# DogRog/no-time-to-train

Hardware: NVIDIA B200
Metric: matching_stage_images_per_s (higher is better)
Workload: dtype f32

## Files before the change

### no-time-to-train_b200/csrc/api.cu

```cuda
#include <cstdio>
#include <cstdlib>
#include <cstring>
#include <mutex>

#include "common.cuh"

namespace nttt {

int launch_lowres_pack(const float*, int, int, int, float, float, uint32_t*, int32_t*, int32_t*, int32_t*, int32_t*,
                       const float*, float, const float* const*, cudaStream_t, float* stab_score = nullptr);
int launch_multimask_select(const float*, int, int, int, const ChunkTable&, int, size_t, const float**, float*,
                            cudaStream_t);
int launch_project_masks(const AxisTable&, const AxisTable&, const uint32_t*, const int32_t*, int, int, int, int, int,
                         void*, int, bool, cudaStream_t, const int32_t* perm = nullptr, uint32_t* active = nullptr);
int launch_pool_order(const int32_t*, int, int, int32_t*, cudaStream_t);
int launch_normalize_split(const float*, int, const int32_t*, int, int, int, float*, void*, bool, cudaStream_t,
                           const int32_t* perm = nullptr);
int launch_gemm_tc(const void*, int, const void*, int, float*, int, int, int, int, int, size_t, int*, cudaStream_t,
                   bool low_latency = false, const uint32_t* a_active = nullptr, const uint8_t* b_nonfinite = nullptr);
int gemm_tc_pick_splits(int, int, int, int);
int launch_split_rows(const float*, int, int, int, int, int, void*, cudaStream_t);
int launch_split_transpose(const float*, int, int, int, int, int, void*, cudaStream_t, uint8_t* nonfinite = nullptr);
int launch_normalize_rows(const float*, int, const int32_t*, int, int, float*, bool, cudaStream_t);
int launch_proto_prepare(const float*, int, int, int, float*, cudaStream_t);
int launch_top1(const float*, int, size_t, float*, int, int, int, float*, int32_t*, cudaStream_t);
int launch_neg_top1(const float*, int, size_t, const float*, int, size_t, int, int, int, float, float*, float*, int32_t*,
                    cudaStream_t);
size_t nms_workspace_bytes(int n);
int launch_box_nms(const int32_t*, const float*, const int32_t*, const float*, int, float, int, int32_t*, int32_t*,
                   int32_t*, int32_t*, void*, size_t, float, int, cudaStream_t);
int launch_upsample_pack(const AxisTable&, const AxisTable&, const float*, const uint32_t*, const int32_t*,
                         const int32_t*, int, int, const int32_t*, const int32_t*, int, int, int, uint32_t*, int32_t*,
                         int32_t*, int32_t*, int32_t*, const float* const*, cudaStream_t, int, int, uint32_t* bits_t = nullptr,
                         bool* wrote_t = nullptr, bool t_only = false, bool low_latency = false, int32_t* zero2 = nullptr);
int32_t* ios_pair_counters(void* ws, int max_sel);
size_t upsample_scratch_bytes(int max_sel, int oh, int ow);
int launch_unpack_sparse(const uint32_t*, const int32_t*, const int32_t*, const int32_t*, int, int, int, uint8_t*,
                         int32_t*, cudaStream_t, bool tr = false);
int launch_unpack(const uint32_t*, const int32_t*, const int32_t*, const int32_t*, int, int, int, uint8_t*,
                  cudaStream_t, bool tr = false);
size_t ios_workspace_bytes(int max_sel);
int launch_mask_ios(const uint32_t*, const int32_t*, const int32_t*, const int32_t*, const int32_t*, const int32_t*,
                    int, int, int, const int32_t*, const float*, int, float*, int32_t*, void*, bool, cudaStream_t,
                    const uint32_t* bits_t = nullptr, bool counters_zeroed = false);
int launch_decay_rank(const float*, const int32_t*, const float*, const int32_t*, const int32_t*, int, int,
                      const int32_t*, const int32_t*, int64_t*, float*, int64_t*, int32_t*, int32_t*, int32_t*, float*,
                      cudaStream_t);
int launch_rle_encode(const uint32_t*, const int32_t*, const int32_t*, const int32_t*, int, int, int, int, int, uint32_t*,
                      int32_t*, uint8_t*, int32_t*, cudaStream_t, bool tr = false);
int launch_rle_compact(const uint8_t*, const int32_t*, int, int, uint8_t*, long long, cudaStream_t);
int launch_fill_pool(const float*, const float*, int, int, int, int, int, int, float*, float*, float*, int, cudaStream_t);
int launch_fill_scatter(const float*, const float*, const float*, const int32_t*, int, int, int, float*, float*, float*,
                        cudaStream_t);
int launch_fill_finalize(const float*, const float*, int, int, int, float*, float*, cudaStream_t);

extern int g_pack_persistent;
static thread_local char g_cuda_err[512] = "";
std::atomic<unsigned long long> g_launches{0};
thread_local bool t_low_latency = false;
thread_local bool t_chain_break = false;

cudaError_t set_dyn_smem_impl(const void* fn, int bytes) {
  struct Entry { const void* fn; int dev; int bytes; };
  static std::mutex mu;
  static Entry table[256];
  static int n = 0;
  int dev = 0;
  cudaError_t e = cudaGetDevice(&dev);
  if (e != cudaSuccess) return e;
  std::lock_guard<std::mutex> lock(mu);
  Entry* hit = nullptr;
  for (int i = 0; i < n; ++i)
    if (table[i].fn == fn && table[i].dev == dev) { hit = &table[i]; break; }
  if (hit && hit->bytes >= bytes) return cudaSuccess;
  e = cudaFuncSetAttribute(fn, cudaFuncAttributeMaxDynamicSharedMemorySize, bytes);
  if (e != cudaSuccess) return e;
  if (hit) hit->bytes = bytes;
  else if (n < 256) table[n++] = Entry{fn, dev, bytes};
  return cudaSuccess;
}

int cuda_fail(cudaError_t e, const char* what) {
  snprintf(g_cuda_err, sizeof(g_cuda_err), "%s: %s (%s)", what, cudaGetErrorString(e), cudaGetErrorName(e));
  return (e == cudaErrorNoDevice || e == cudaErrorInsufficientDriver) ? NTTT_ENODEVICE : NTTT_ECUDA;
}

struct Carver {
  char* base;
  size_t off = 0;
  explicit Carver(void* p) : base(static_cast<char*>(p)) {}
  template <typename T>
  T* take(size_t count) {
    off = align_up(off, 256);
    T* p = base ? reinterpret_cast<T*>(base + off) : nullptr;
    off += sizeof(T) * count;
    return p;
  }
};

inline int pad64(int k) { return (k + 63) / 64 * 64; }

constexpr int kPoolSplitsMax = 2;
constexpr int kPoolSplits = 1;
static int pool_contract(const float* proj, const float* feat, int n, int e, int c, float* sums, void* a_split,
                         void* b_split, int* n_partials, cudaStream_t s, bool low_latency = false, bool b_ready = false,
                         const uint32_t* a_active = nullptr, uint8_t* b_nonfinite = nullptr) {
  const int ep = pad64(e);
  int err = proj ? launch_split_rows(proj, e, n, e, ep, 0, a_split, s) : NTTT_OK;
  if (err) return err;
  err = b_ready ? NTTT_OK : launch_split_transpose(feat, c, c, e, ep, 1, b_split, s, a_active ? b_nonfinite : nullptr);
  if (err) return err;
  return launch_gemm_tc(a_split, 3 * ep, b_split, 3 * ep, sums, c, n, c, 3 * ep, low_latency ? kPoolSplitsMax : kPoolSplits,
                        (size_t)n * c, n_partials, s, low_latency, a_active, a_active ? b_nonfinite : nullptr);
}

static int normalize_rows(const float* sums, int n_partials, const int32_t* area, int n, int c, float* obj_feats,
                          void* a_split, bool* split_done, bool nan_empty, cudaStream_t s, const int32_t* perm = nullptr) {
  *split_done = a_split &&
                launch_normalize_split(sums, n_partials, area, n, c, pad64(c), obj_feats, a_split, nan_empty, s, perm) == 1;
  if (*split_done) return NTTT_OK;
  if (perm) return NTTT_EINVAL;
  return launch_normalize_rows(sums, n_partials, area, n, c, obj_feats, nan_empty, s);
}

static bool projection_supported(int in_size, int out_size) {
  return in_size > 0 && 2 * ((out_size + in_size - 1) / in_size) + 2 <= kMaxScatter;
}

constexpr int kMaxSimSplits = 8;
static size_t sim_partial_floats(int n, int cols, int c) {
  int sp = gemm_tc_pick_splits(n, cols, 3 * pad64(c), 148);
  if (sp > kMaxSimSplits) sp = kMaxSimSplits;
  return (size_t)sp * n * cols;
}

static int sim_top1(const float* obj_feats, const float* proto, const float* proto_neg, int l_neg, float sigma, int n,
                    int c, int n_cls, float* sim, float* partials, float* partials_neg, float* top_score,
                    int32_t* top_label, void* a_split, void* b_split, bool a_ready, int sm_count, cudaStream_t s,
                    void* p_split = nullptr, bool p_ready = false) {
  const int cp = pad64(c);
  int err = a_ready ? NTTT_OK : launch_split_rows(obj_feats, c, n, c, cp, 0, a_split, s);
  if (err) return err;
  void* pb = p_split ? p_split : b_split;
  err = p_ready ? NTTT_OK : launch_split_rows(proto, c, n_cls, c, cp, 1, pb, s);
  if (err) return err;
  int want = gemm_tc_pick_splits(n, n_cls, 3 * cp, sm_count < 148 ? sm_count : 148);
  if (want > kMaxSimSplits) want = kMaxSimSplits;
  if (!t_low_latency) want = 1;
  const size_t stride = (size_t)n * n_cls;
  int splits = 1;
  err = launch_gemm_tc(a_split, 3 * cp, pb, 3 * cp, partials, n_cls, n, n_cls, 3 * cp, want, stride, &splits, s);
  if (err) return err;
  if (!proto_neg) return launch_top1(partials, splits, stride, sim, n_cls, n, n_cls, top_score, top_label, s);
  const int cols = n_cls * l_neg;
  err = launch_split_rows(proto_neg, c, cols, c, cp, 1, b_split, s);
  if (err) return err;
  int want_n = gemm_tc_pick_splits(n, cols, 3 * cp, sm_count < 148 ? sm_count : 148);
  if (want_n > kMaxSimSplits) want_n = kMaxSimSplits;
  if (!t_low_latency) want_n = 1;
  const size_t stride_n = (size_t)n * cols;
  int splits_n = 1;
  err = launch_gemm_tc(a_split, 3 * cp, b_split, 3 * cp, partials_neg, cols, n, cols, 3 * cp, want_n, stride_n, &splits_n,
                       s);
  if (err) return err;
  return launch_neg_top1(partials, splits, stride, partials_neg, splits_n, stride_n, n, n_cls, l_neg, sigma, sim,
                         top_score, top_label, s);
}

// ... 488 lines not shown
  L.sim_part = cv.take<float>(sim_partial_floats(n, n_cls, c));
  L.sim_part_neg = cv.take<float>(l_neg > 0 ? sim_partial_floats(n, n_cls * l_neg, c) : 1);
  {
    const size_t kmax = (size_t)3 * (pad64(eh * ew) > pad64(c) ? pad64(eh * ew) : pad64(c));
    size_t rows_b = (size_t)(c > n_cls ? c : n_cls);
    if ((size_t)n_cls * (l_neg > 0 ? l_neg : 0) > rows_b) rows_b = (size_t)n_cls * l_neg;
    L.a_split = cv.take<char>(2 * (size_t)n * kmax);
    L.b_split = cv.take<char>(2 * rows_b * kmax);
    L.p_split = cv.take<char>(2 * (size_t)n_cls * 3 * pad64(c));
    L.pool_perm = cv.take<int32_t>(n > 0 ? n : 1);
    L.pool_active = cv.take<uint32_t>(n > 0 ? n : 1);
    L.b_nonfinite = cv.take<uint8_t>((size_t)(pad64(eh * ew) / 64) * ((c + 31) / 32));
  }
  L.top_score = cv.take<float>(n);
  L.top_label = cv.take<int32_t>(n);
  L.nms_ws_bytes = nms_workspace_bytes(n > 0 ? n : 1);
  L.nms_ws = cv.take<char>(L.nms_ws_bytes);
  L.keep = cv.take<int32_t>(max_sel > 0 ? max_sel : 1);
  L.sel = cv.take<int32_t>(max_sel > 0 ? max_sel : 1);
  L.bits_full = cv.take<uint32_t>((size_t)max_sel * oh * ((ow + 31) / 32));
  L.bits_t = cv.take<uint32_t>((size_t)max_sel * oh * ((ow + 31) / 32));
  L.rect = cv.take<int32_t>((size_t)max_sel * 4);
  L.area_full = cv.take<int32_t>(max_sel > 0 ? max_sel : 1);
  L.box_full = cv.take<int32_t>((size_t)max_sel * 4);
  L.scratch = cv.take<int32_t>(upsample_scratch_bytes(max_sel > 0 ? max_sel : 1, oh, ow) / sizeof(int32_t) + 1);
  L.ios = cv.take<float>(max_sel > 0 ? max_sel : 1);
  L.ios_ws = cv.take<char>(ios_workspace_bytes(max_sel > 0 ? max_sel : 1));
  L.out_slot = cv.take<int32_t>(num_out > 0 ? num_out : 1);
  L.mask_ptr = cv.take<const float*>(n > 0 ? n : 1);
  L.plane_score = cv.take<float>(n > 0 ? n : 1);
  L.total = align_up(cv.off, 256);
  return L;
}

size_t nttt_match_workspace_bytes(int n, int lr_h, int lr_w, int eh, int ew, int c, int n_cls, int ori_h, int ori_w,
                                  int max_sel) {
  if (n < 0 || lr_h <= 0 || lr_w <= 0 || eh <= 0 || ew <= 0 || c <= 0 || n_cls <= 0 || ori_h <= 0 || ori_w <= 0 ||
      max_sel < 0)
    return 0;
  return carve(nullptr, n, lr_h, lr_w, eh, ew, c, n_cls, ori_h, ori_w, max_sel, max_sel, 0).total;
}

size_t nttt_match_workspace_bytes_neg(int n, int lr_h, int lr_w, int eh, int ew, int c, int n_cls, int ori_h, int ori_w,
                                      int max_sel, int l_neg) {
  if (n < 0 || lr_h <= 0 || lr_w <= 0 || eh <= 0 || ew <= 0 || c <= 0 || n_cls <= 0 || ori_h <= 0 || ori_w <= 0 ||
      max_sel < 0 || l_neg < 0)
    return 0;
  return carve(nullptr, n, lr_h, lr_w, eh, ew, c, n_cls, ori_h, ori_w, max_sel, max_sel, l_neg).total;
}

int nttt_match_image(nttt_ctx* ctx, const nttt_match_args* a, void* stream) {
  if (!ctx || !a) return NTTT_EINVAL;
  if (a->n < 0 || a->lr_h <= 0 || a->lr_w <= 0 || a->eh <= 0 || a->ew <= 0 || a->c <= 0 || a->n_cls <= 0 ||
      a->ori_h <= 0 || a->ori_w <= 0 || a->num_out_instance < 0 || a->max_sel < 0)
    return NTTT_EINVAL;
  if (!a->counts || !a->workspace) return NTTT_EINVAL;
  cudaStream_t s = (cudaStream_t)stream;
  const int n = a->n, max_sel = a->max_sel, num_out = a->num_out_instance;
  if (n == 0 || max_sel == 0) {
    NTTT_CUDA(cudaMemsetAsync(a->counts, 0, 4 * sizeof(int32_t), s));
    return NTTT_OK;
  }
  const bool multi = a->n_multi > 1;
  const bool chunked = multi && a->logits_chunks_host;
  const bool want_rle = a->rle_chars != nullptr;
  if ((!a->logits && !chunked) || (!multi && !a->pred_ious) || !a->tar_feat || !a->proto ||
      (!a->out_masks && !want_rle) || !a->out_boxes || !a->out_scores || !a->out_labels || !a->out_index)
    return NTTT_EINVAL;
  if (want_rle && (!a->rle_counts || !a->rle_n_counts || !a->rle_n_chars || a->rle_cap_counts <= 0 || a->rle_cap_chars <= 0))
    return NTTT_EINVAL;
  if (multi && (!a->multi_ious || a->multi_first < 0 || a->multi_first >= a->n_multi)) return NTTT_EINVAL;
  const int l_neg = a->proto_neg ? a->l_neg : 0;
  if (a->proto_neg && (a->l_neg <= 0 || !(a->sigma > 0.0f))) return NTTT_EINVAL;
  MatchLayout L = carve(a->workspace, n, a->lr_h, a->lr_w, a->eh, a->ew, a->c, a->n_cls, a->ori_h, a->ori_w, max_sel,
                        num_out, l_neg);
  if (a->workspace_bytes < L.total) return NTTT_EWORKSPACE;
  if (!projection_supported(a->ew, a->lr_w) || !projection_supported(a->eh, a->lr_h)) return NTTT_EUNSUPPORTED;
  float* obj_feats = a->obj_feats ? a->obj_feats : L.obj_feats;
  float* sim = a->sim ? a->sim : L.sim;
  int32_t* sel = a->sel ? a->sel : L.sel;
  float* ios = a->ios ? a->ios : L.ios;
  struct LaunchMode {
    bool prev;
    explicit LaunchMode(bool v) : prev(nttt::t_low_latency) { nttt::t_low_latency = v; }
    ~LaunchMode() { nttt::t_low_latency = prev; }
  } launch_mode(a->low_latency != 0);
  ++ctx->epoch;
  AxisTable px, py, ux, uy;
  int err = ctx->axis(a->ew, a->lr_w, s, &px);
  if (err) return err;
  if ((err = ctx->axis(a->eh, a->lr_h, s, &py))) return err;
  if ((err = ctx->axis(a->lr_w, a->ori_w, s, &ux))) return err;
  if ((err = ctx->axis(a->lr_h, a->ori_h, s, &uy))) return err;
  const int e = a->eh * a->ew;

  ctx->n_ev = 0;
#define NTTT_MARK()                                                              \
  do {                                                                           \
    if (ctx->profile) { NTTT_CUDA(cudaEventRecord(ctx->ev[ctx->n_ev], s)); ++ctx->n_ev; } \
  } while (0)
#ifdef NTTT_ABLATE
  int stage_no = 0;
#define NTTT_STOP_CHECK() if (ctx->stop_after > 0 && ++stage_no >= ctx->stop_after) return NTTT_OK
#else
#define NTTT_STOP_CHECK() (void)0
#endif
#define NTTT_STEP_QUIET(call) \
  do {                        \
    err = (call);             \
    if (err) return err;      \
  } while (0)
#define NTTT_STEP(call)                                        \
  do {                                                         \
    err = (call);                                              \
    if (err) return err;                                       \
    NTTT_MARK();                                               \
    NTTT_STOP_CHECK();                                         \
  } while (0)
  const float* const* mask_ptr = nullptr;
  const float* pred_ious = a->pred_ious;
  if (multi) {
    ChunkTable ct;
    const float* one = a->logits;
    err = chunked ? make_chunk_table(a->logits_chunks_host, a->n_chunks, a->chunk_prompts, n, &ct)
                  : make_chunk_table(&one, 1, n, n, &ct);
    if (err) return err;
    if ((err = launch_multimask_select(a->multi_ious, n, a->n_multi, a->multi_first, ct, chunked ? a->chunk_prompts : n,
                                       (size_t)a->lr_h * a->lr_w, L.mask_ptr, L.plane_score, s)))
      return err;
    mask_ptr = L.mask_ptr;
    pred_ious = L.plane_score;
  }
  NTTT_MARK();
  const bool forked = a->low_latency != 0 && ctx->side_ready();
  struct SideJoin {
    cudaStream_t s;
    cudaEvent_t ev = nullptr;
    ~SideJoin() { if (ev) cudaStreamWaitEvent(s, ev, 0); }
  } side_join{s};
  if (forked) {
    NTTT_CUDA(cudaEventRecord(ctx->ev_fork, s));
    NTTT_CUDA(cudaStreamWaitEvent(ctx->side, ctx->ev_fork, 0));
    err = launch_split_transpose(a->tar_feat, a->c, a->c, e, pad64(e), 1, L.b_split, ctx->side);
    if (err) return err;
    err = launch_split_rows(a->proto, a->c, a->n_cls, a->c, pad64(a->c), 1, L.p_split, ctx->side);
    if (err) return err;
    NTTT_CUDA(cudaEventRecord(ctx->ev_join, ctx->side));
    side_join.ev = ctx->ev_join;
  }
  NTTT_STEP(launch_lowres_pack(a->logits, n, a->lr_h, a->lr_w, 0.0f, 1.0f, L.bits_lr, L.area_lr, L.box_lr, nullptr,
                               L.flags, a->filter_iou ? pred_ious : nullptr, a->iou_thr, mask_ptr, s));
  const bool ordered = !a->low_latency && ctx->pool_order && n > 128 && n <= 8192 && pad64(e) / 64 <= 32 &&
                       (a->c == 384 || a->c == 768 || a->c == 1024 || a->c == 1536);
  if (ordered) NTTT_STEP_QUIET(launch_pool_order(L.box_lr, n, a->lr_h, L.pool_perm, s));
  NTTT_STEP(launch_project_masks(px, py, L.bits_lr, L.box_lr, n, a->lr_h, a->lr_w, a->eh, a->ew, L.a_split, pad64(e),
                                 true, s, ordered ? L.pool_perm : nullptr, ordered ? L.pool_active : nullptr));
  int n_partials = 1;
  if (forked) {
    NTTT_CUDA(cudaStreamWaitEvent(s, ctx->ev_join, 0));
    side_join.ev = nullptr;
    nttt::t_chain_break = true;
  }
  NTTT_STEP(pool_contract(nullptr, a->tar_feat, n, e, a->c, L.sums, L.a_split, L.b_split, &n_partials, s,
                          a->low_latency != 0, forked, ordered ? L.pool_active : nullptr, L.b_nonfinite));
  bool a_ready = false;
  NTTT_STEP(normalize_rows(L.sums, n_partials, L.area_lr, n, a->c, obj_feats, L.a_split, &a_ready,
                           a->proto_neg != nullptr, s, ordered ? L.pool_perm : nullptr));
  NTTT_STEP(sim_top1(obj_feats, a->proto, a->proto_neg, l_neg, a->sigma, n, a->c, a->n_cls, a->sim, L.sim_part,
                     L.sim_part_neg, L.top_score, L.top_label, L.a_split, L.b_split, a_ready, ctx->sm_count, s, L.p_split,
                     forked));
  NTTT_STEP(launch_box_nms(L.box_lr, pred_ious, L.top_label, L.top_score, n, a->nms_thr, max_sel, L.keep,
                           a->counts + 0, sel, a->counts + 1, L.nms_ws, L.nms_ws_bytes, a->iou_thr, a->filter_iou, s));
  bool wrote_t = false;
  NTTT_STEP(launch_upsample_pack(ux, uy, a->logits, L.bits_lr, L.box_lr, L.flags, a->lr_h, a->lr_w, sel,
                                 a->counts + 1, max_sel, a->ori_h, a->ori_w, L.bits_full, L.rect, L.area_full,
                                 L.box_full, L.scratch, mask_ptr, s, ctx->upsample_stage_floats, ctx->sm_count, L.bits_t,
                                 &wrote_t, true, a->low_latency != 0, ios_pair_counters(L.ios_ws, max_sel)));
  const uint32_t* packed = wrote_t ? L.bits_t : L.bits_full;
  NTTT_STEP(launch_mask_ios(L.bits_full, L.rect, L.area_full, L.box_full, sel, a->counts + 1, max_sel, a->ori_h,
                            a->ori_w, L.top_label, obj_feats, a->c, ios, a->ios_inter, L.ios_ws, false, s,
                            wrote_t ? L.bits_t : nullptr, wrote_t && a->low_latency != 0));
  NTTT_STEP(launch_decay_rank(L.top_score, L.top_label, ios, sel, a->counts + 1, max_sel, num_out, L.box_full,
                              L.area_full,
                              a->out_boxes, a->out_scores, a->out_labels, a->out_index, L.out_slot, a->counts + 2,
                              nullptr, s));
  if (!a->out_masks)
    NTTT_MARK();
  else if (a->out_prev_rect)
    NTTT_STEP(launch_unpack_sparse(packed, L.rect, L.out_slot, a->counts + 2, num_out, a->ori_h, a->ori_w,
                                   a->out_masks, a->out_prev_rect, s, wrote_t));
  else
    NTTT_STEP(launch_unpack(packed, L.rect, L.out_slot, a->counts + 2, num_out, a->ori_h, a->ori_w, a->out_masks,
                            s, wrote_t));
  if (want_rle)
    NTTT_STEP(launch_rle_encode(packed, L.rect, L.out_slot, a->counts + 2, num_out, a->ori_h, a->ori_w,
                                a->rle_cap_counts, a->rle_cap_chars, a->rle_counts, a->rle_n_counts, a->rle_chars,
                                a->rle_n_chars, s, wrote_t));
  else
    NTTT_MARK();
#undef NTTT_STEP
#undef NTTT_STOP_CHECK
#undef NTTT_MARK
  return NTTT_OK;
}

}
```

### no-time-to-train_b200/csrc/lowres.cu

```cuda
#include <cuda_bf16.h>
#include <stdlib.h>

#include <algorithm>

#include "common.cuh"

namespace nttt {

constexpr int kPackThreads = 256;
constexpr int kPackBlock = kPackThreads + 32;
constexpr int kPackStages = 4;
constexpr int kPackStageF4 = 4 * kPackThreads;
constexpr int kPackStageBytes = kPackStageF4 * 16;

__device__ __forceinline__ uint32_t pk_smem_u32(const void* p) { return (uint32_t)__cvta_generic_to_shared(p); }
__device__ __forceinline__ void pk_mbar_init(uint64_t* bar, uint32_t count) {
  asm volatile("mbarrier.init.shared::cta.b64 [%0], %1;" ::"r"(pk_smem_u32(bar)), "r"(count));
}
__device__ __forceinline__ void pk_mbar_expect_tx(uint32_t bar_addr, uint32_t bytes) {
  asm volatile("mbarrier.arrive.expect_tx.shared::cta.b64 _, [%0], %1;" ::"r"(bar_addr), "r"(bytes) : "memory");
}
__device__ __forceinline__ void pk_mbar_arrive(uint32_t bar_addr) {
  asm volatile("mbarrier.arrive.shared::cta.b64 _, [%0];" ::"r"(bar_addr) : "memory");
}
// ... 568 lines not shown
  const int size = hi - lo;
  const float lo_m_center = __fsub_rn((float)lo, center);
  float total = 0.0f;
  float* wi = w + (size_t)i * taps;
  for (int j = 0; j < size; ++j) {
    float x = __fmul_rn(__fadd_rn(__fadd_rn((float)j, lo_m_center), 0.5f), invscale);
    x = fabsf(x);
    const float v = x < 1.0f ? __fsub_rn(1.0f, x) : 0.0f;
    wi[j] = v;
    total = __fadd_rn(total, v);
  }
  if (total != 0.0f)
    for (int j = 0; j < size; ++j) wi[j] = __fdiv_rn(wi[j], total);
  for (int j = size; j < taps; ++j) wi[j] = 0.0f;
  xmin[i] = lo;
  xsize[i] = size;
}

__global__ void aa_transpose_kernel(int in_size, int out_size, int taps, const int32_t* xmin, const int32_t* xsize,
                                    const float* w, int32_t* t_lo, int32_t* t_len, float* t_w, float* t_cum) {
  const int e = blockIdx.x * blockDim.x + threadIdx.x;
  if (e >= in_size) return;
  int lo = -1, hi = -1;
  for (int x = 0; x < out_size; ++x) {
    if (e >= xmin[x] && e < xmin[x] + xsize[x]) {
      if (lo < 0) lo = x;
      hi = x;
    }
  }
  const int len = lo < 0 ? 0 : hi - lo + 1;
  t_lo[e] = max(lo, 0);
  t_len[e] = len;
  for (int t = 0; t < kMaxScatter; ++t) {
    const int x = lo + t;
    float v = 0.0f;
    if (lo >= 0 && x <= hi && e >= xmin[x] && e < xmin[x] + xsize[x]) v = w[(size_t)x * taps + (e - xmin[x])];
    t_w[(size_t)e * kMaxScatter + t] = v;
  }
  float c = 0.0f;
  t_cum[(size_t)e * (kMaxScatter + 1)] = 0.0f;
  for (int t = 0; t < kMaxScatter; ++t) {
    c += t_w[(size_t)e * kMaxScatter + t];
    t_cum[(size_t)e * (kMaxScatter + 1) + t + 1] = c;
  }
}

__global__ void aa_group_kernel(int out_size, const int32_t* xmin, const int32_t* xsize, int32_t* grp_of,
                                int32_t* grp_start) {
  if (blockIdx.x != 0 || threadIdx.x != 0) return;
  int g = -1, run = 0;
  for (int i = 0; i < out_size; ++i) {
    const bool same = i > 0 && xmin[i] == xmin[i - 1] && xsize[i] == xsize[i - 1] && run < kGrpMax;
    if (!same) { ++g; grp_start[g] = i; run = 0; }
    grp_of[i] = g;
    ++run;
  }
  for (int k = g + 1; k <= out_size; ++k) grp_start[k] = out_size;
}

__global__ void aa_pack_kernel(int out_size, int out_pad, int taps, const int32_t* xmin, const int32_t* xsize,
                               const float* w, uint32_t* pk_span, float2* pk_w) {
  const int i = blockIdx.x * blockDim.x + threadIdx.x;
  if (i >= out_pad) return;
  uint32_t span = 0;
  float2 e = make_float2(0.f, 0.f);
  if (i < out_size) {
    const int cs = xsize[i];
    const float* wi = w + (size_t)i * taps;
    span = (uint32_t)xmin[i] | ((uint32_t)cs << 16);
    e.x = cs > 0 ? wi[0] : 0.0f;
    e.y = cs > 1 ? wi[1] : 0.0f;
  }
  pk_span[i] = span;
  pk_w[i] = e;
}

static bool aa_spans_within_two(int in_size, int out_size) {
  if (in_size > out_size) return false;
  const float scale = (float)in_size / (float)out_size;
  for (int i = 0; i < out_size; ++i) {
    volatile float center = scale * ((float)i + 0.5f);
    volatile float a = center - 1.0f, b = center + 1.0f;
    const int lo = std::max((int)(a + 0.5f), 0), hi = std::min((int)(b + 0.5f), in_size);
    if (hi - lo > 2) return false;
  }
  return true;
}

int build_axis_table(AxisTable& t, int in_size, int out_size, cudaStream_t s) {
  t.in_size = in_size;
  t.out_size = out_size;
  t.taps = aa_max_taps(in_size, out_size);
  const bool packed = in_size < 65536 && aa_spans_within_two(in_size, out_size);
  const int out_pad = (out_size + 31) / 32 * 32;
  size_t off = 0;
  auto take = [&](size_t bytes) { const size_t o = off; off = align_up(off + bytes, 256); return o; };
  const size_t o_xmin = take(sizeof(int32_t) * out_size), o_xsize = take(sizeof(int32_t) * out_size);
  const size_t o_w = take(sizeof(float) * (size_t)out_size * t.taps);
  const size_t o_tlo = take(sizeof(int32_t) * in_size), o_tlen = take(sizeof(int32_t) * in_size);
  const size_t o_tw = take(sizeof(float) * (size_t)in_size * kMaxScatter);
  const size_t o_tcum = take(sizeof(float) * (size_t)in_size * (kMaxScatter + 1));
  const size_t o_gof = take(sizeof(int32_t) * out_size), o_gst = take(sizeof(int32_t) * ((size_t)out_size + 1));
  const size_t o_pks = packed ? take(sizeof(uint32_t) * (size_t)out_pad) : 0;
  const size_t o_pkw = packed ? take(sizeof(float2) * (size_t)out_pad) : 0;
  char* slab = nullptr;
  NTTT_CUDA(cudaMalloc(&slab, off));
  t.slab = slab;
  t.xmin = reinterpret_cast<int32_t*>(slab + o_xmin);
  t.xsize = reinterpret_cast<int32_t*>(slab + o_xsize);
  t.w = reinterpret_cast<float*>(slab + o_w);
  t.t_lo = reinterpret_cast<int32_t*>(slab + o_tlo);
  t.t_len = reinterpret_cast<int32_t*>(slab + o_tlen);
  t.t_w = reinterpret_cast<float*>(slab + o_tw);
  t.t_cum = reinterpret_cast<float*>(slab + o_tcum);
  t.grp_of = reinterpret_cast<int32_t*>(slab + o_gof);
  t.grp_start = reinterpret_cast<int32_t*>(slab + o_gst);
  t.pk_span = packed ? reinterpret_cast<uint32_t*>(slab + o_pks) : nullptr;
  t.pk_w = packed ? reinterpret_cast<float2*>(slab + o_pkw) : nullptr;
  aa_table_kernel<<<ceil_div(out_size, 128), 128, 0, s>>>(in_size, out_size, t.taps, t.xmin, t.xsize, t.w);
  NTTT_LAUNCH_CHECK();
  aa_transpose_kernel<<<ceil_div(in_size, 128), 128, 0, s>>>(in_size, out_size, t.taps, t.xmin, t.xsize, t.w, t.t_lo,
                                                            t.t_len, t.t_w, t.t_cum);
  NTTT_LAUNCH_CHECK();
  aa_group_kernel<<<1, 32, 0, s>>>(out_size, t.xmin, t.xsize, t.grp_of, t.grp_start);
  NTTT_LAUNCH_CHECK();
  if (packed) {
    aa_pack_kernel<<<ceil_div(out_pad, 128), 128, 0, s>>>(out_size, out_pad, t.taps, t.xmin, t.xsize, t.w, t.pk_span,
                                                             t.pk_w);
    NTTT_LAUNCH_CHECK();
  }
  return NTTT_OK;
}

void free_axis_table(AxisTable& t) {
  if (t.slab) cudaFree(t.slab);
  t = AxisTable{};
}

constexpr int kProjThreads = 256;

struct ProjTables {
  const int32_t* x_lo; const int32_t* x_len; const float* x_cum;
  const int32_t* y_lo; const int32_t* y_len; const float* y_w;
};

__device__ __forceinline__ void split_bf16_pair(float x, __nv_bfloat16& hi, __nv_bfloat16& lo) {
  hi = __float2bfloat16_rn(x);
  lo = __float2bfloat16_rn(x - __bfloat162float(hi));
}

constexpr int kCum = kMaxScatter + 1;
constexpr int kProjRows = 64;

template <typename F>
__device__ __forceinline__ void warp_range(int n, F flag, int& lo, int& hi) {
  const int lane = lane_id();
  const uint32_t b0 = __ballot_sync(kFull, lane < n && flag(lane));
  const uint32_t b1 = __ballot_sync(kFull, lane + 32 < n && flag(lane + 32));
  lo = b0 ? __ffs(b0) - 1 : (b1 ? 32 + __ffs(b1) - 1 : 1);
  hi = b1 ? 63 - __clz(b1) : (b0 ? 31 - __clz(b0) : 0);
}

template <bool kSplit>
__global__ void __launch_bounds__(kProjThreads)
project_masks_kernel(const uint32_t* __restrict__ bits, const int32_t* __restrict__ box, int n_masks, int h,
                     int words_per_row, int eh, int ew, ProjTables t, void* __restrict__ out, int stride_or_kp,
                     const int32_t* __restrict__ perm, uint32_t* __restrict__ active) {
  chain_wait();
  extern __shared__ uint32_t smem[];
  const int rc = min(h, kProjRows);
  int* s_xlo = reinterpret_cast<int*>(smem);
  int* s_xlen = s_xlo + ew;
  int* s_ylo = s_xlen + ew;
  int* s_ylen = s_ylo + eh;
  uint32_t* s_bits = reinterpret_cast<uint32_t*>(s_ylen + eh);
  float* s_row = reinterpret_cast<float*>(s_bits + rc * words_per_row);
  float* s_acc = s_row + rc * ew;
  const int lane = lane_id(), warp = warp_id();
  constexpr int kWarps = kProjThreads / 32;
  if (eh > 64 || ew > 64) return;
  for (int i = threadIdx.x; i < ew; i += kProjThreads) { s_xlo[i] = t.x_lo[i]; s_xlen[i] = min(t.x_len[i], kMaxScatter); }
  for (int i = threadIdx.x; i < eh; i += kProjThreads) { s_ylo[i] = t.y_lo[i]; s_ylen[i] = min(t.y_len[i], kMaxScatter); }
  for (int n = blockIdx.x; n < n_masks; n += gridDim.x) {
  __syncthreads();
  const int4 b = reinterpret_cast<const int4*>(box)[n];
  const uint32_t* src = bits + (size_t)n * h * words_per_row;
  const bool empty = (b.x | b.y | b.z | b.w) == 0 && (src[0] & 1u) == 0;
  const int orow = perm ? perm[n] : n;
  const int top = b.y, bottom = b.w, left = b.x, right = b.z;

  {
    const size_t row_bytes = kSplit ? (size_t)3 * stride_or_kp * 2 : (size_t)stride_or_kp * 4;
    char* o = static_cast<char*>(out) + (size_t)orow * row_bytes;
    if ((row_bytes & 15) == 0) {
      for (int i = threadIdx.x; i < (int)(row_bytes >> 4); i += kProjThreads)
        reinterpret_cast<uint4*>(o)[i] = make_uint4(0, 0, 0, 0);
    } else {
      for (int i = threadIdx.x; i < (int)(row_bytes >> 2); i += kProjThreads) reinterpret_cast<uint32_t*>(o)[i] = 0;
    }
  }
  if (empty) {
    if (active && threadIdx.x == 0) active[orow] = 0u;
    continue;
  }
  const int nrows = bottom - top + 1;
  int ex_lo, ex_hi, ey_lo, ey_hi;
  warp_range(ew, [&](int e) { return s_xlo[e] <= right && s_xlo[e] + s_xlen[e] > left; }, ex_lo, ex_hi);
  warp_range(eh, [&](int e) { return s_ylo[e] <= bottom && s_ylo[e] + s_ylen[e] > top; }, ey_lo, ey_hi);
  const int nex = ex_hi - ex_lo + 1;
  if (nex <= 0 || ey_hi < ey_lo) {
    if (active && threadIdx.x == 0) active[orow] = 0u;
    continue;
  }
  if (active && warp == 0) {
    uint32_t m = 0;
    if (eh * ew > 32 * 64) {
      m = 0xffffffffu;
    } else {
      for (int ey = ey_lo + lane; ey <= ey_hi; ey += 32) {
        const int k0 = (ey * ew + ex_lo) >> 6, k1 = (ey * ew + ex_hi) >> 6;
        m |= (k1 - k0 >= 31 ? 0xffffffffu : ((2u << (k1 - k0)) - 1u)) << k0;
      }
    }
    m = __reduce_or_sync(kFull, m);
    if (lane == 0) active[orow] = m;
  }
  for (int ey = ey_lo + warp; ey <= ey_hi; ey += kWarps)
    for (int ex = ex_lo + lane; ex <= ex_hi; ex += 32) s_acc[ey * ew + ex] = 0.0f;

  for (int cb = 0; cb < nrows; cb += rc) {
    const int rows_c = min(rc, nrows - cb);
    const int ctop = top + cb;
    if (cb > 0) __syncthreads();
    for (int i = threadIdx.x; i < rows_c * words_per_row; i += kProjThreads) s_bits[i] = src[ctop * words_per_row + i];
    __syncthreads();
    for (int yy = warp; yy < rows_c; yy += kWarps) {
      const uint32_t* row = s_bits + yy * words_per_row;
      for (int ex = ex_lo + lane; ex <= ex_hi; ex += 32) {
        const int lo = s_xlo[ex], len = s_xlen[ex];
        const int w0 = lo >> 5, sh = lo & 31;
        const uint32_t wa = row[w0];
        const uint32_t wb = (w0 + 1 < words_per_row) ? row[w0 + 1] : 0u;
        uint32_t f = __funnelshift_r(wa, wb, sh);
        f &= (len >= 32) ? 0xffffffffu : ((1u << len) - 1u);
        const float* cw = t.x_cum + ex * kCum;
        float acc = 0.0f;
        while (f) {
          const int a = __ffs(f) - 1;
          const uint32_t g = ~(f >> a);
          const int run = g ? __ffs(g) - 1 : 32 - a;
          acc += __ldg(cw + a + run) - __ldg(cw + a);
          f = (a + run >= 32) ? 0u : (f >> (a + run)) << (a + run);
        }
        s_row[yy * nex + (ex - ex_lo)] = acc;
      }
    }
    __syncthreads();
    for (int ey = ey_lo + warp; ey <= ey_hi; ey += kWarps) {
      const int lo = s_ylo[ey], len = s_ylen[ey];
      const float* wv = t.y_w + ey * kMaxScatter;
      const int ta = max(max(top - lo, 0), ctop - lo), tb = min(min(bottom - lo + 1, len), ctop + rows_c - lo);
      if (ta >= tb) continue;
      for (int ex = ex_lo + lane; ex <= ex_hi; ex += 32) {
        float acc = s_acc[ey * ew + ex];
        for (int q = ta; q < tb; ++q) acc = fmaf(__ldg(wv + q), s_row[(lo + q - ctop) * nex + (ex - ex_lo)], acc);
        s_acc[ey * ew + ex] = acc;
      }
    }
  }
  for (int ey = ey_lo + warp; ey <= ey_hi; ey += kWarps) {
    for (int ex = ex_lo + lane; ex <= ex_hi; ex += 32) {
      const float acc = s_acc[ey * ew + ex];
      const int item = ey * ew + ex;
      if (kSplit) {
        __nv_bfloat16 hi, lo16;
        split_bf16_pair(acc, hi, lo16);
        __nv_bfloat16* o = static_cast<__nv_bfloat16*>(out) + (size_t)orow * 3 * stride_or_kp;
        o[item] = hi;
        o[stride_or_kp + item] = hi;
        o[2 * stride_or_kp + item] = lo16;
      } else {
        static_cast<float*>(out)[(size_t)orow * stride_or_kp + item] = acc;
      }
    }
  }
  }
}

static size_t project_smem_bytes(int h, int w, int eh, int ew) {
  const int rc = h < kProjRows ? h : kProjRows;
  return sizeof(int) * 2 * (size_t)(ew + eh) + sizeof(uint32_t) * (size_t)rc * (w / 32) +
         sizeof(float) * (size_t)rc * ew + sizeof(float) * (size_t)eh * ew;
}

int launch_project_masks(const AxisTable& tx, const AxisTable& ty, const uint32_t* bits, const int32_t* box, int n,
                         int h, int w, int eh, int ew, void* out, int out_stride, bool split, cudaStream_t s,
                         const int32_t* perm, uint32_t* active) {
  if (n <= 0) return NTTT_OK;
  if (w % 32 != 0 || eh > 64 || ew > 64) return NTTT_EUNSUPPORTED;
  const size_t smem = project_smem_bytes(h, w, eh, ew);
  if (smem > 200 * 1024) return NTTT_EUNSUPPORTED;
  ProjTables t{tx.t_lo, tx.t_len, tx.t_cum, ty.t_lo, ty.t_len, ty.t_w};
  const int grid = t_low_latency ? n : min(n, 2 * current_sm_count());
  if (split) {
    if (smem > 48 * 1024)
      NTTT_CUDA(set_dyn_smem(project_masks_kernel<true>, (int)smem));
    launch_chain(project_masks_kernel<true>, grid, kProjThreads, smem, s, bits, box, n, h, w / 32, eh, ew, t, out, out_stride, perm,
                 active);
  } else {
    if (smem > 48 * 1024)
      NTTT_CUDA(set_dyn_smem(project_masks_kernel<false>, (int)smem));
    project_masks_kernel<false><<<grid, kProjThreads, smem, s>>>(bits, box, n, h, w / 32, eh, ew, t, out, out_stride, perm, active);
  }
  NTTT_LAUNCH_CHECK();
  return NTTT_OK;
}

constexpr int kOrderBins = 64 * 64;
__global__ void __launch_bounds__(1024)
pool_order_kernel(const int32_t* __restrict__ box, int n, int h, int32_t* __restrict__ perm) {
  chain_wait();
  __shared__ int s_hist[kOrderBins];
  __shared__ int s_warp[33];
  const int tid = threadIdx.x, lane = tid & 31, warp = tid >> 5;
  for (int i = tid; i < kOrderBins; i += 1024) s_hist[i] = 0;
  __syncthreads();
  const int shift = 32 - __clz((h - 1) >> 6);
  constexpr int kMaxPer = 8;
  int key[kMaxPer], rank[kMaxPer];
#pragma unroll
  for (int q = 0; q < kMaxPer; ++q) {
    const int i = q * 1024 + tid;
    key[q] = -1;
    if (i < n) {
      const int4 b = reinterpret_cast<const int4*>(box)[i];
      const uint32_t t0 = (uint32_t)min(b.y >> shift, 63), t1 = (uint32_t)min(b.w >> shift, 63);
      uint32_t code = 0;
#pragma unroll
      for (int bit = 0; bit < 6; ++bit) code |= (((t0 >> bit) & 1u) << (2 * bit + 1)) | (((t1 >> bit) & 1u) << (2 * bit));
      key[q] = (int)code;
      rank[q] = atomicAdd(&s_hist[key[q]], 1);
    }
  }
  __syncthreads();
  int c0 = s_hist[4 * tid], c1 = s_hist[4 * tid + 1], c2 = s_hist[4 * tid + 2], c3 = s_hist[4 * tid + 3];
  const int mine = c0 + c1 + c2 + c3;
  int inc = mine;
#pragma unroll
  for (int o = 1; o < 32; o <<= 1) {
    const int up = __shfl_up_sync(kFull, inc, o);
    if (lane >= o) inc += up;
  }
  if (lane == 31) s_warp[warp] = inc;
  __syncthreads();
  if (warp == 0) {
    const int w = s_warp[lane];
    int winc = w;
#pragma unroll
    for (int o = 1; o < 32; o <<= 1) {
      const int up = __shfl_up_sync(kFull, winc, o);
      if (lane >= o) winc += up;
    }
    s_warp[lane] = winc - w;
  }
  __syncthreads();
  const int base = s_warp[warp] + inc - mine;
  s_hist[4 * tid] = base;
  s_hist[4 * tid + 1] = base + c0;
  s_hist[4 * tid + 2] = base + c0 + c1;
  s_hist[4 * tid + 3] = base + c0 + c1 + c2;
  __syncthreads();
#pragma unroll
  for (int q = 0; q < kMaxPer; ++q) {
    const int i = q * 1024 + tid;
    if (i < n) perm[i] = s_hist[key[q]] + rank[q];
  }
}

int launch_pool_order(const int32_t* box, int n, int h, int32_t* perm, cudaStream_t s) {
  if (n <= 0) return NTTT_OK;
  if (n > 8192) return NTTT_EUNSUPPORTED;
  launch_chain(pool_order_kernel, 1, 1024, 0, s, box, n, h, perm);
  NTTT_LAUNCH_CHECK();
  return NTTT_OK;
}

}
```

Baseline: 12500.

## Fuse pool-order permutation computation into project_masks kernel

Removes the separate single-CTA pool_order kernel. Every project_masks CTA now redundantly builds the histogram and prefix sum in shared memory, reusing the working buffer, and derives a stable rank per mask with warp ballots over earlier keys. The permutation row for each CTA's own masks is cached in shared memory, and perm is written for later stages. This saves a serialized launch on the chain but makes every CTA repeat the ordering work and an O(n) rank scan per mask. It also adds a minimum-blocks launch bound of 5, which may limit registers.

```diff
diff --git a/no-time-to-train_b200/csrc/api.cu b/no-time-to-train_b200/csrc/api.cu
--- a/no-time-to-train_b200/csrc/api.cu
+++ b/no-time-to-train_b200/csrc/api.cu
@@ -12,8 +12,7 @@
 int launch_multimask_select(const float*, int, int, int, const ChunkTable&, int, size_t, const float**, float*,
                             cudaStream_t);
 int launch_project_masks(const AxisTable&, const AxisTable&, const uint32_t*, const int32_t*, int, int, int, int, int,
-                         void*, int, bool, cudaStream_t, const int32_t* perm = nullptr, uint32_t* active = nullptr);
-int launch_pool_order(const int32_t*, int, int, int32_t*, cudaStream_t);
+                         void*, int, bool, cudaStream_t, int32_t* perm = nullptr, uint32_t* active = nullptr);
 int launch_normalize_split(const float*, int, const int32_t*, int, int, int, float*, void*, bool, cudaStream_t,
                            const int32_t* perm = nullptr);
 int launch_gemm_tc(const void*, int, const void*, int, float*, int, int, int, int, int, size_t, int*, cudaStream_t,
@@ -808,7 +807,6 @@
                                L.flags, a->filter_iou ? pred_ious : nullptr, a->iou_thr, mask_ptr, s));
   const bool ordered = !a->low_latency && ctx->pool_order && n > 128 && n <= 8192 && pad64(e) / 64 <= 32 &&
                        (a->c == 384 || a->c == 768 || a->c == 1024 || a->c == 1536);
-  if (ordered) NTTT_STEP_QUIET(launch_pool_order(L.box_lr, n, a->lr_h, L.pool_perm, s));
   NTTT_STEP(launch_project_masks(px, py, L.bits_lr, L.box_lr, n, a->lr_h, a->lr_w, a->eh, a->ew, L.a_split, pad64(e),
                                  true, s, ordered ? L.pool_perm : nullptr, ordered ? L.pool_active : nullptr));
   int n_partials = 1;
diff --git a/no-time-to-train_b200/csrc/lowres.cu b/no-time-to-train_b200/csrc/lowres.cu
--- a/no-time-to-train_b200/csrc/lowres.cu
+++ b/no-time-to-train_b200/csrc/lowres.cu
@@ -744,6 +744,63 @@
 constexpr int kCum = kMaxScatter + 1;
 constexpr int kProjRows = 64;
 
+constexpr int kOrderBins = 64 * 64;
+
+__device__ __forceinline__ int order_key(const int4& b, int shift) {
+  const uint32_t t0 = (uint32_t)min(b.y >> shift, 63), t1 = (uint32_t)min(b.w >> shift, 63);
+  uint32_t code = 0;
+#pragma unroll
+  for (int bit = 0; bit < 6; ++bit) code |= (((t0 >> bit) & 1u) << (2 * bit + 1)) | (((t1 >> bit) & 1u) << (2 * bit));
+  return (int)code;
+}
+
+template <int kThreads>
+__device__ void order_masks(const int32_t* __restrict__ box, int n, int h, int* s_hist, uint16_t* s_key, int* s_orow,
+                            int32_t* __restrict__ perm) {
+  constexpr int kPer = kOrderBins / kThreads, kWarps = kThreads / 32;
+  __shared__ int s_wsum[kWarps];
+  const int tid = threadIdx.x, lane = tid & 31, warp = tid >> 5;
+  for (int i = tid; i < kOrderBins; i += kThreads) s_hist[i] = 0;
+  __syncthreads();
+  const int shift = 32 - __clz((h - 1) >> 6);
+  for (int i = tid; i < n; i += kThreads) {
+    const int k = order_key(reinterpret_cast<const int4*>(box)[i], shift);
+    s_key[i] = (uint16_t)k;
+    atomicAdd(&s_hist[k], 1);
+  }
+  __syncthreads();
+  int* hb = s_hist + tid * kPer;
+  int mine = 0;
+#pragma unroll 1
+  for (int q = 0; q < kPer; ++q) mine += hb[q];
+  int inc = mine;
+#pragma unroll
+  for (int o = 1; o < 32; o <<= 1) {
+    const int up = __shfl_up_sync(kFull, inc, o);
+    if (lane >= o) inc += up;
+  }
+  if (lane == 31) s_wsum[warp] = inc;
+  __syncthreads();
+  int base = inc - mine;
+  for (int w = 0; w < warp; ++w) base += s_wsum[w];
+#pragma unroll 1
+  for (int q = 0; q < kPer; ++q) {
+    const int c = hb[q];
+    hb[q] = base;
+    base += c;
+  }
+  __syncthreads();
+  for (int k = warp; blockIdx.x + k * gridDim.x < n; k += kWarps) {
+    const int m = blockIdx.x + k * gridDim.x, key = s_key[m];
+    int rank = 0;
+    for (int j0 = 0; j0 < m; j0 += 32) rank += __popc(__ballot_sync(kFull, j0 + lane < m && s_key[j0 + lane] == key));
+    if (lane == 0) {
+      s_orow[k] = s_hist[key] + rank;
+      perm[m] = s_hist[key] + rank;
+    }
+  }
+}
+
 template <typename F>
 __device__ __forceinline__ void warp_range(int n, F flag, int& lo, int& hi) {
   const int lane = lane_id();
@@ -754,10 +811,10 @@
 }
 
 template <bool kSplit>
-__global__ void __launch_bounds__(kProjThreads)
+__global__ void __launch_bounds__(kProjThreads, 5)
 project_masks_kernel(const uint32_t* __restrict__ bits, const int32_t* __restrict__ box, int n_masks, int h,
                      int words_per_row, int eh, int ew, ProjTables t, void* __restrict__ out, int stride_or_kp,
-                     const int32_t* __restrict__ perm, uint32_t* __restrict__ active) {
+                     int32_t* __restrict__ perm, uint32_t* __restrict__ active) {
   chain_wait();
   extern __shared__ uint32_t smem[];
   const int rc = min(h, kProjRows);
@@ -765,7 +822,9 @@
   int* s_xlen = s_xlo + ew;
   int* s_ylo = s_xlen + ew;
   int* s_ylen = s_ylo + eh;
-  uint32_t* s_bits = reinterpret_cast<uint32_t*>(s_ylen + eh);
+  int* s_orow = s_ylen + eh;
+  const int per_cta = perm ? (n_masks + gridDim.x - 1) / gridDim.x : 0;
+  uint32_t* s_bits = reinterpret_cast<uint32_t*>(s_orow + per_cta);
   float* s_row = reinterpret_cast<float*>(s_bits + rc * words_per_row);
   float* s_acc = s_row + rc * ew;
   const int lane = lane_id(), warp = warp_id();
@@ -773,12 +832,15 @@
   if (eh > 64 || ew > 64) return;
   for (int i = threadIdx.x; i < ew; i += kProjThreads) { s_xlo[i] = t.x_lo[i]; s_xlen[i] = min(t.x_len[i], kMaxScatter); }
   for (int i = threadIdx.x; i < eh; i += kProjThreads) { s_ylo[i] = t.y_lo[i]; s_ylen[i] = min(t.y_len[i], kMaxScatter); }
+  if (perm)
+    order_masks<kProjThreads>(box, n_masks, h, reinterpret_cast<int*>(s_bits),
+                              reinterpret_cast<uint16_t*>(reinterpret_cast<int*>(s_bits) + kOrderBins), s_orow, perm);
   for (int n = blockIdx.x; n < n_masks; n += gridDim.x) {
   __syncthreads();
   const int4 b = reinterpret_cast<const int4*>(box)[n];
   const uint32_t* src = bits + (size_t)n * h * words_per_row;
   const bool empty = (b.x | b.y | b.z | b.w) == 0 && (src[0] & 1u) == 0;
-  const int orow = perm ? perm[n] : n;
+  const int orow = perm ? s_orow[(n - blockIdx.x) / gridDim.x] : n;
   const int top = b.y, bottom = b.w, left = b.x, right = b.z;
 
   {
@@ -879,21 +941,22 @@
   }
 }
 
-static size_t project_smem_bytes(int h, int w, int eh, int ew) {
+static size_t project_smem_bytes(int h, int w, int eh, int ew, int order_n = 0, int per_cta = 0) {
   const int rc = h < kProjRows ? h : kProjRows;
-  return sizeof(int) * 2 * (size_t)(ew + eh) + sizeof(uint32_t) * (size_t)rc * (w / 32) +
-         sizeof(float) * (size_t)rc * ew + sizeof(float) * (size_t)eh * ew;
+  const size_t work = sizeof(uint32_t) * (size_t)rc * (w / 32) + sizeof(float) * (size_t)rc * ew + sizeof(float) * (size_t)eh * ew;
+  const size_t order = order_n > 0 ? sizeof(int) * (size_t)kOrderBins + sizeof(uint16_t) * (size_t)order_n : 0;
+  return sizeof(int) * (2 * (size_t)(ew + eh) + per_cta) + std::max(work, order);
 }
 
 int launch_project_masks(const AxisTable& tx, const AxisTable& ty, const uint32_t* bits, const int32_t* box, int n,
                          int h, int w, int eh, int ew, void* out, int out_stride, bool split, cudaStream_t s,
-                         const int32_t* perm, uint32_t* active) {
+                         int32_t* perm, uint32_t* active) {
   if (n <= 0) return NTTT_OK;
-  if (w % 32 != 0 || eh > 64 || ew > 64) return NTTT_EUNSUPPORTED;
-  const size_t smem = project_smem_bytes(h, w, eh, ew);
+  if (w % 32 != 0 || eh > 64 || ew > 64 || (perm && n > 8192)) return NTTT_EUNSUPPORTED;
+  const int grid = t_low_latency ? n : min(n, 2 * current_sm_count());
+  const size_t smem = project_smem_bytes(h, w, eh, ew, perm ? n : 0, perm ? ceil_div(n, grid) : 0);
   if (smem > 200 * 1024) return NTTT_EUNSUPPORTED;
   ProjTables t{tx.t_lo, tx.t_len, tx.t_cum, ty.t_lo, ty.t_len, ty.t_w};
-  const int grid = t_low_latency ? n : min(n, 2 * current_sm_count());
   if (split) {
     if (smem > 48 * 1024)
       NTTT_CUDA(set_dyn_smem(project_masks_kernel<true>, (int)smem));
@@ -908,73 +971,4 @@
   return NTTT_OK;
 }
 
-constexpr int kOrderBins = 64 * 64;
-__global__ void __launch_bounds__(1024)
-pool_order_kernel(const int32_t* __restrict__ box, int n, int h, int32_t* __restrict__ perm) {
-  chain_wait();
-  __shared__ int s_hist[kOrderBins];
-  __shared__ int s_warp[33];
-  const int tid = threadIdx.x, lane = tid & 31, warp = tid >> 5;
-  for (int i = tid; i < kOrderBins; i += 1024) s_hist[i] = 0;
-  __syncthreads();
-  const int shift = 32 - __clz((h - 1) >> 6);
-  constexpr int kMaxPer = 8;
-  int key[kMaxPer], rank[kMaxPer];
-#pragma unroll
-  for (int q = 0; q < kMaxPer; ++q) {
-    const int i = q * 1024 + tid;
-    key[q] = -1;
-    if (i < n) {
-      const int4 b = reinterpret_cast<const int4*>(box)[i];
-      const uint32_t t0 = (uint32_t)min(b.y >> shift, 63), t1 = (uint32_t)min(b.w >> shift, 63);
-      uint32_t code = 0;
-#pragma unroll
-      for (int bit = 0; bit < 6; ++bit) code |= (((t0 >> bit) & 1u) << (2 * bit + 1)) | (((t1 >> bit) & 1u) << (2 * bit));
-      key[q] = (int)code;
-      rank[q] = atomicAdd(&s_hist[key[q]], 1);
-    }
-  }
-  __syncthreads();
-  int c0 = s_hist[4 * tid], c1 = s_hist[4 * tid + 1], c2 = s_hist[4 * tid + 2], c3 = s_hist[4 * tid + 3];
-  const int mine = c0 + c1 + c2 + c3;
-  int inc = mine;
-#pragma unroll
-  for (int o = 1; o < 32; o <<= 1) {
-    const int up = __shfl_up_sync(kFull, inc, o);
-    if (lane >= o) inc += up;
-  }
-  if (lane == 31) s_warp[warp] = inc;
-  __syncthreads();
-  if (warp == 0) {
-    const int w = s_warp[lane];
-    int winc = w;
-#pragma unroll
-    for (int o = 1; o < 32; o <<= 1) {
-      const int up = __shfl_up_sync(kFull, winc, o);
-      if (lane >= o) winc += up;
-    }
-    s_warp[lane] = winc - w;
-  }
-  __syncthreads();
-  const int base = s_warp[warp] + inc - mine;
-  s_hist[4 * tid] = base;
-  s_hist[4 * tid + 1] = base + c0;
-  s_hist[4 * tid + 2] = base + c0 + c1;
-  s_hist[4 * tid + 3] = base + c0 + c1 + c2;
-  __syncthreads();
-#pragma unroll
-  for (int q = 0; q < kMaxPer; ++q) {
-    const int i = q * 1024 + tid;
-    if (i < n) perm[i] = s_hist[key[q]] + rank[q];
-  }
-}
-
-int launch_pool_order(const int32_t* box, int n, int h, int32_t* perm, cudaStream_t s) {
-  if (n <= 0) return NTTT_OK;
-  if (n > 8192) return NTTT_EUNSUPPORTED;
-  launch_chain(pool_order_kernel, 1, 1024, 0, s, box, n, h, perm);
-  NTTT_LAUNCH_CHECK();
-  return NTTT_OK;
-}
-
-}
+}
```

Result: slower. 11690, median of 6 (-6.5%).
